# Starfish-develop/Starfish

Hardware: AMD Instinct MI355X
Metric: log-likelihood evals/sec, 4096-pixel order, batch=128 walkers (higher is better)
Workload: dtype f64; 1 GPU; cfg2: synthetic single order N_pix=4096, 8 eigenspectra, M=27, N_f=8192, 1 global + 1 local kernel, all 13 parameters thawed, batch=128 walkers per GPU; global_batch=128, units_per_gpu=128, parallelism=(order x walker) units sharded x1, one process per GPU, no data-path collective

## Files before the change

starfish_amd/csrc/sf_abi.cpp:

```cpp
#include "sf_stages.h"

sf_emu_args emu_args(sf_ctx* c, const sf_model_desc* mdl, const double* d_params, const Work& w, double* d_mu, double* d_cov,
                     double* d_Lw, int* d_info) {
    sf_emu_args e;
    e.params = d_params;
    e.pstride = sf_param_stride(c, mdl);
    e.off_grid = 6;
    e.m = c->m;
    e.M = c->M;
    e.P = c->P;
    e.grid = c->grid.as<double>();
    e.variances = c->variances.as<double>();
    e.lengthscales = c->lengthscales.as<double>();
    e.gmin = c->gmin.as<double>();
    e.gmax = c->gmax.as<double>();
    e.alpha = c->alpha.as<double>();
    e.LinvT = c->Linv.as<double>();
    e.zscratch = w.zs;
    e.kbuf = w.kv;
    e.mu = d_mu;
    e.cov = d_cov;
    e.Lw = d_Lw;
    e.info = d_info;
    return e;
// ... 256 lines not shown
    hipStream_t s = (hipStream_t)stream;
    prof_count_call();
    {
        ProfScope ps(s, PS_TRANSFORM);
        rc = run_transforms(c, mdl, B, d_params, w, nullptr, nullptr, nullptr, nullptr, true, s);
        if (rc) return rc;
    }
    {
        ProfScope ps(s, PS_FILL);
        rc = fill_dense(c, mdl, B, d_params, w, d_cov, ld, stride, lower_only ? 1 : 0, add_jitter ? 1 : 0, c->n, s);
        if (rc) return rc;
    }
    return export_info(d_info, w, B, s);
}

sf_fill_args loglike_fill_args(sf_ctx* c, const sf_model_desc* mdl, const double* d_params, const Work& w, const Layout& L,
                               int fp) {
    sf_fill_args f = fill_args(c, mdl, d_params, w);
    f.C = w.C;
    f.lda = L.lda;
    f.stride = (int64_t)L.npad * L.lda;
    f.lower_only = 1;
    f.add_jitter = 1;
    f.gtab = w.gtab;
    f.tilemap = w.tilemap;
    f.tilelist = w.tilelist;
    f.tilecount = w.tilecount;
    f.list_cap = (int)tilemap_bytes(L);
    f.fp = fp;
    f.nt128 = (L.npad + fp + 127) / 128;
    return f;
}
int loglike_factor_finish(const Work& w, const Layout& L, int fp, int units, double* ltbuf, double* d_lnl, int* d_info,
                          hipStream_t s, sf_exec* ex) {
    const int64_t stride = (int64_t)L.npad * L.lda;
    int rc;
    {
        ProfScope ps(s, PS_POTRF);
        sf_gen_args gen;
        gen.Y = w.Y;
        gen.mpad = L.mpad;
        gen.ldy = L.npad;
        gen.tilemap = w.tilemap;
        gen.fp = fp;
        gen.nt128 = (L.npad + fp + 127) / 128;
        rc = sf_launch_potrf(w.C, L.npad, L.lda, stride, units, w.info_c, ltbuf, w.resid, L.npad, s, &gen, ex);
        if (rc) return rc;
    }
    {
        ProfScope ps(s, PS_SOLVE);
        rc = sf_launch_logdet_z(w.C, L.npad, L.lda, stride, units, w.resid, L.npad, w.logdet, w.sqmah, s);
        if (rc) return rc;
        rc = sf_launch_finish(units, w.logdet, w.sqmah, w.info_e, w.info_c, d_lnl, d_info, s);
        if (rc) return rc;
    }
    return SF_OK;
}

extern "C" int sf_loglike_batch(sf_ctx* c, const sf_model_desc* mdl, int B, const double* d_params,
                                double* d_lnl, double* d_logdet, double* d_sqmah, double* d_resid,
                                double* d_log_scale, int* d_info, void* d_work, size_t work_bytes,
                                void* stream) {
    Work w;
    int rc = open_call(c, mdl, B, d_work, work_bytes, true, &w);
    if (rc) return rc;
    if (!d_lnl) {
        sf_set_error("sf_loglike_batch: d_lnl is required");
        return SF_EINVAL;
    }
    hipStream_t s = (hipStream_t)stream;
    prof_count_call();
    const Layout L = layout_of(c);
    {
        ProfScope ps(s, PS_TRANSFORM);
        rc = run_transforms(c, mdl, B, d_params, w, nullptr, nullptr, d_resid, d_log_scale, true, s);
        if (rc) return rc;
    }
    const int fp = sf_potrf_front_pad(c->npad, B);
    {
        ProfScope ps(s, PS_FILL);
        rc = sf_launch_fill(loglike_fill_args(c, mdl, d_params, w, L, fp), B, s);
        if (rc) return rc;
    }
    rc = loglike_factor_finish(w, L, fp, B, w.ltbuf, d_lnl, d_info, s, &c->exec);
    if (rc) return rc;
    return export_logdet_sqmah(d_logdet, d_sqmah, w, B, s);
}
```

starfish_amd/csrc/sf_chol_seq.h:

```cpp
#pragma once
#include "sf_chol_host.h"
#include "sf_chol_diag.h"
#include "sf_chol_panel.h"
#include "sf_chol_wide.h"

static int sf_check_front_pad(int fp, int n) {
    if (fp != 0 && (fp != 64 || n % GT != 64)) {
        sf_set_error("potrf: front pad %d does not fit n = %d", fp, n);
        return SF_EINVAL;
    }
    return SF_OK;
}

template <class Args>
static void sf_park(Args& g, const sf_potrf_scratch& ws) {
    g.Sout = ws.T;
    g.sS = ws.sT;
    g.ldS = SF_LDT;
}
static double sf_slab_rows(int n, int row0, int nslab, int step) {
    double rows = 0.0;
    for (int i = 0; i < nslab; ++i) {
        const int r0 = row0 + i * step * GT;
        rows += (n - r0 < GT) ? n - r0 : GT;
// ... 103 lines not shown
    g.slab_step = step;
    g.Wt0 = ws.Wslot(k);
    g.Wt1 = ws.Wslot(k + 1);
    g.sW = ws.sW;
    if (park) sf_park(g, ws);
    const long long nblk = (long long)nslab * batch;
    SF_TRY(sf_check_grid(nblk));
#ifdef SF_TUNING
    if (stamps.t && stamps.n < 64) {
        stamps.k[stamps.n] = k * 1000 + nslab;
        g.stamps = stamps.t + 16 * stamps.n++;
    }
#endif
    const double rows = sf_slab_rows(n, g.row0, nslab, step);
    const double kk = g.k0 > fp ? g.k0 - fp : 0;
    const double flops = (2.0 * kk * rows * GT + 2.0 * (kk + GT) * rows * GT + 2.0 * (rows * GT * (double)GT + (double)GT * rows * GT)) * batch;
    void* tok;
    sf_prof_gemm_begin(st, flops, &tok);
    if (g.rhs)
        hipLaunchKernelGGL(k_chol_panel_w<true>, dim3((unsigned)nblk), dim3(1024), SF_PANELW_LDS, st, g);
    else
        hipLaunchKernelGGL(k_chol_panel_w<false>, dim3((unsigned)nblk), dim3(1024), SF_PANELW_LDS, st, g);
    sf_prof_gemm_end(tok);
    SF_LAUNCH_CHECK();
    return SF_OK;
}

static int sf_diag_step(const sf_potrf_scratch& ws, double* A, int lda, int64_t stride, double* rhs, int ldr, int* info, int n, int k,
                        double* Wt, int fp, hipStream_t st) {
    const int k0 = k * GT;
    const int pw = (n - k0 < GT) ? n - k0 : GT;
    return sf_launch_diag128(ws.T, ws.sT, pw, info, k0 - fp, rhs ? rhs + k0 : nullptr, ldr, A + (int64_t)k0 * lda + k0, lda, stride, Wt,
                             ws.sW, ws.batch, st, k == 0 ? fp : 0);
}

struct sf_narrow_events {
    hipEvent_t d, rest[2];
};
static int sf_narrow_step(const sf_panel_args& base, const sf_potrf_scratch& ws, sf_exec* ex, int* info, int k, double* Wt, hipStream_t c,
                          const hipStream_t gs[2], const hipEvent_t last[2], hipEvent_t* e_top, sf_narrow_events* ev) {
    const int n = base.n, fp = base.fp, nt = (n + GT - 1) / GT;
    const int k0 = k * GT;
    const int pw = (n - k0 < GT) ? n - k0 : GT;
    *ev = {};
    SF_TRY(sf_diag_step(ws, base.C, base.lda, base.sC, base.rhs, base.ldr, info, n, k, Wt, fp, c));
    if (k + 1 >= nt) return SF_OK;
    SF_TRY(sf_exec_event(ex, &ev->d));
    SF_HIP(hipEventRecord(ev->d, c));
    const int gk = (k + 1) & 1;
    if (e_top && sf_panel_split(k0, pw, fp, ws.batch) > 1) {
        if (*e_top) SF_HIP(hipStreamWaitEvent(gs[gk], *e_top, 0));
        SF_TRY(sf_panel_step(base, ws, k0, pw, (k + 1) * GT, 1, 1, Wt, true, gs[gk], 0, 1));
        hipEvent_t e_part;
        SF_TRY(sf_exec_event(ex, &e_part));
        SF_HIP(hipEventRecord(e_part, gs[gk]));
        SF_HIP(hipStreamWaitEvent(c, e_part, 0));
        SF_TRY(sf_panel_step(base, ws, k0, pw, (k + 1) * GT, 1, 1, Wt, true, c, 0, 2));
    } else {
        if (last[gk]) SF_HIP(hipStreamWaitEvent(c, last[gk], 0));
        SF_TRY(sf_panel_step(base, ws, k0, pw, (k + 1) * GT, 1, 1, Wt, true, c, 0, 0));
    }
    if (e_top) {
        SF_TRY(sf_exec_event(ex, e_top));
        SF_HIP(hipEventRecord(*e_top, c));
    }
    for (int g = 0; g < 2; ++g) {
        const int first = k + 2 + (((k + 2) & 1) != g);
        if (first >= nt) continue;
        const int cnt = (nt - 1 - first) / 2 + 1;
        SF_HIP(hipStreamWaitEvent(gs[g], ev->d, 0));
        SF_TRY(sf_panel_step(base, ws, k0, pw, first * GT, cnt, 2, Wt, false, gs[g], 1 + g, 0));
        SF_TRY(sf_exec_event(ex, &ev->rest[g]));
        SF_HIP(hipEventRecord(ev->rest[g], gs[g]));
    }
    return SF_OK;
}

static int sf_launch_potrf_v2(double* A, int n, int lda, int64_t stride, int* info, const sf_potrf_scratch& ws, double* rhs,
                              int ldr, hipStream_t s, const sf_gen_args* gen, sf_exec* ex, int fp) {
    const int batch = ws.batch;
    SF_HIP(hipMemsetAsync(info, 0, sizeof(int) * (size_t)batch, s));
    SF_TRY(sf_exec_prepare(ex));
    constexpr int G = 2;
    hipStream_t c = ex->side;
    const hipStream_t gs[G] = {s, ex->grp[0]};
    SF_TRY(sf_exec_fork(ex, s, {c, gs[1]}));

    const sf_panel_args base = sf_panel_frame<sf_panel_args>(A, n, lda, stride, rhs, ldr, gen, fp);
    const int nt = (n + GT - 1) / GT;
    SF_TRY(sf_panel_step(base, ws, 0, 0, 0, 1, 1, nullptr, true, c, 0, 0));
    hipEvent_t e_epi = nullptr;
    hipEvent_t e_rest[G] = {};
    hipEvent_t e_rest_prev[G] = {};
    for (int k = 0; k < nt; ++k) {
        for (int g = 0; g < G; ++g)
            if (e_rest_prev[g]) SF_HIP(hipStreamWaitEvent(c, e_rest_prev[g], 0));
        sf_narrow_events ev;
        SF_TRY(sf_narrow_step(base, ws, ex, info, k, ws.Wbuf(k & 1), c, gs, e_rest, &e_epi, &ev));
        for (int g = 0; g < G; ++g) {
            e_rest_prev[g] = e_rest[g];
            if (ev.rest[g]) e_rest[g] = ev.rest[g];
        }
    }
    SF_TRY(sf_exec_join(ex, s, c, {e_rest[1]}));
    return SF_OK;
}

static int sf_launch_potrf_v3(double* A, int n, int lda, int64_t stride, int* info, const sf_potrf_scratch& ws, double* rhs,
                              int ldr, hipStream_t s, const sf_gen_args* gen, sf_exec* ex, bool half, int fp) {
    const int batch = ws.batch;
    static sf_dev_once attr_once;
    SF_CHECK(sf_lds_limit_once(&attr_once, 160 * 1024, {(const void*)k_chol_panel_w<true>, (const void*)k_chol_panel_w<false>}));
    SF_HIP(hipMemsetAsync(info, 0, sizeof(int) * (size_t)batch, s));
    SF_TRY(sf_exec_prepare(ex));
    hipStream_t c = ex->side, xa = ex->side;
    SF_TRY(sf_exec_fork(ex, s, {c, xa, ex->grp[0]}));
    const int nt = (n + GT - 1) / GT;

    const sf_panel_args base = sf_panel_frame<sf_panel_args>(A, n, lda, stride, rhs, ldr, gen, fp);
    const sf_panelw_args wbase = sf_panel_frame<sf_panelw_args>(A, n, lda, stride, rhs, ldr, gen, fp);
    sf_wide_stamps stamps;
    SF_TRY(sf_wide_stamps_begin(stamps));
    auto diag = [&](int k) -> int { return sf_diag_step(ws, A, lda, stride, rhs, ldr, info, n, k, ws.Wslot(k), fp, c); };

    SF_TRY(sf_panel_step(base, ws, 0, 0, 0, 1, 1, nullptr, true, c, 0, 0));
    const hipStream_t bs[2] = {s, ex->grp[0]};
    hipEvent_t e_A = nullptr;
    hipEvent_t e_last[2] = {nullptr, nullptr};
    std::vector<hipEvent_t> readers[4];
    auto wait_readers = [&](int slot) -> int {
        for (hipEvent_t e : readers[slot]) SF_HIP(hipStreamWaitEvent(c, e, 0));
        readers[slot].clear();
        return SF_OK;
    };
    int k = 0;
    for (; k < nt; k += 2) {
        if (k + 2 >= nt) break;
        if (half && k >= (nt / 4) * 2 && k > 0) break;
        if (e_A) SF_HIP(hipStreamWaitEvent(c, e_A, 0));
        SF_TRY(wait_readers(k & 3));
        SF_TRY(diag(k));
        SF_TRY(sf_panel_step(base, ws, k * GT, GT, (k + 1) * GT, 1, 1, ws.Wslot(k), true, c, 0, 0));
        SF_TRY(wait_readers((k + 1) & 3));
        SF_TRY(diag(k + 1));
        hipEvent_t e_chain;
        SF_TRY(sf_exec_event(ex, &e_chain));
        SF_HIP(hipEventRecord(e_chain, c));
        const int na = (nt - (k + 2) < 2) ? nt - (k + 2) : 2;
        SF_HIP(hipStreamWaitEvent(xa, e_chain, 0));
        for (int g = 0; g < 2; ++g)
            if (e_last[g]) SF_HIP(hipStreamWaitEvent(xa, e_last[g], 0));
        SF_TRY(sf_panel_step_w(wbase, ws, k, k + 2, na, 1, true, xa, stamps));
        SF_TRY(sf_exec_event(ex, &e_A));
        SF_HIP(hipEventRecord(e_A, xa));
        readers[k & 3].push_back(e_A);
        readers[(k + 1) & 3].push_back(e_A);
        for (int g = 0; g < 2; ++g) {
            const int first = k + 4 + g;
            if (first >= nt) continue;
            const int cnt = (nt - 1 - first) / 2 + 1;
            SF_HIP(hipStreamWaitEvent(bs[g], e_chain, 0));
            SF_TRY(sf_panel_step_w(wbase, ws, k, first, cnt, 2, false, bs[g], stamps));
            SF_TRY(sf_exec_event(ex, &e_last[g]));
            SF_HIP(hipEventRecord(e_last[g], bs[g]));
            readers[k & 3].push_back(e_last[g]);
            readers[(k + 1) & 3].push_back(e_last[g]);
        }
    }
    for (; k < nt; ++k) {
        if (e_A) {
            SF_HIP(hipStreamWaitEvent(c, e_A, 0));
            for (int g = 0; g < 2; ++g) SF_HIP(hipStreamWaitEvent(bs[g], e_A, 0));
            e_A = nullptr;
        }
        SF_TRY(wait_readers(k & 3));
        sf_narrow_events ev;
        SF_TRY(sf_narrow_step(base, ws, ex, info, k, ws.Wslot(k), c, bs, e_last, nullptr, &ev));
        for (int g = 0; g < 2; ++g)
            if (ev.rest[g]) {
                e_last[g] = ev.rest[g];
                readers[k & 3].push_back(ev.rest[g]);
            }
    }
    SF_TRY(sf_exec_join(ex, s, c, {e_A, e_last[1]}));
    sf_wide_stamps_report(stamps, s);
    return SF_OK;
}
```

starfish_amd/csrc/sf_common.h:

```cpp
#pragma once
#include <hip/hip_runtime.h>
#include <stdint.h>
#include <stddef.h>
#include <stdlib.h>
#include <atomic>
#include <initializer_list>
#include <mutex>
#include "sf_base.h"

#define SF_LEAF 64
#define SF_NB 256
#define SF_MAX_LOCAL 32
#define SF_NF_MIN_VSINI 16
#define SF_NF_MAX_VSINI 65536

typedef double sf_d4 __attribute__((ext_vector_type(4)));

#define SF_HIP(call)                                                                     \
    do {                                                                                 \
        hipError_t e_ = (call);                                                          \
        if (e_ != hipSuccess) {                                                          \
            sf_set_error("%s:%d %s -> %s", __FILE__, __LINE__, #call, hipGetErrorString(e_)); \
            return SF_EHIP;                                                              \
        }                                                                                \
// ... 28 lines not shown
}
static inline int sf_lds_limit_once(sf_dev_once* once, int bytes, std::initializer_list<const void*> kernels) {
    return sf_once_per_device(once, [&]() -> int {
        for (const void* k : kernels) SF_HIP(hipFuncSetAttribute(k, hipFuncAttributeMaxDynamicSharedMemorySize, bytes));
        return SF_OK;
    });
}
#define SF_CHECK(expr)              \
    do {                            \
        const int rc_ = (expr);     \
        if (rc_ != SF_OK) return rc_; \
    } while (0)

#ifdef SF_TUNING
#define SF_TUNE_FLAG(name) (getenv(name) != nullptr)
#define SF_TUNE_INT(name, dflt) (getenv(name) ? atoi(getenv(name)) : (dflt))
#define SF_TUNE_STR(name) (static_cast<const char*>(getenv(name)))
#else
#define SF_TUNE_FLAG(name) (false)
#define SF_TUNE_INT(name, dflt) (dflt)
#define SF_TUNE_STR(name) (static_cast<const char*>(nullptr))
#endif

#ifndef SF_EXEC_GROUPS
#define SF_EXEC_GROUPS 2
#endif
static_assert(SF_EXEC_GROUPS >= 2, "the wide sequence and the multi-order lanes use grp[0]: at least two slab groups");
struct sf_exec {
    int device = -1;
    hipStream_t side = nullptr;
    hipStream_t grp[SF_EXEC_GROUPS - 1] = {};
    hipStream_t aux = nullptr;
    hipEvent_t fork = nullptr, join = nullptr;
    hipEvent_t* pool = nullptr;
    size_t pool_size = 0, pool_cap = 0, used = 0;
};
int sf_exec_prepare(sf_exec* ex);
int sf_exec_event(sf_exec* ex, hipEvent_t* e);
void sf_exec_release(sf_exec* ex);
sf_exec* sf_exec_thread_local(void);

void sf_prof_gemm_begin(hipStream_t s, double flops, void** tok);
void sf_prof_gemm_end(void* tok);

#define SF_LTB_DOUBLES (SF_LEAF * SF_LEAF + SF_LEAF)
#define SF_LDT (SF_NB + 16)
size_t sf_potrf_work_doubles(int n, int batch);
struct sf_gen_args {
    const double* Y;
    int mpad, ldy;
    const unsigned char* tilemap;
    int nt128;
    int fp;
};
int sf_potrf_front_pad(int n, int batch);
int sf_launch_potrf(double* A, int n, int lda, int64_t stride, int batch, int* info, double* work,
                    double* rhs, int ldr, hipStream_t s, const sf_gen_args* gen = nullptr, sf_exec* ex = nullptr);
int sf_band_tiles_lda(int nband);
size_t sf_band_tiles_doubles(int nband, int batch);
int sf_band_tiles_wt(int halfwidth);
int sf_set_persistent_potrf(int enable);
int sf_persistent_potrf_read_status(long long* out8);
int sf_set_cholesky_sequence(int mode);
int sf_launch_logdet_z(const double* L, int n, int lda, int64_t stride, int batch, const double* z, int ldr,
                       double* logdet, double* sqmah, hipStream_t s);
int sf_launch_logdet_sqmah(const double* L, int n, int lda, int64_t stride, int batch,
                           const double* R, int ldr, double* zscratch, double* logdet, double* sqmah, hipStream_t s);
int sf_launch_chol_apply(const double* L, int n, int lda, int64_t stride, int batch, int op, const double* rhs, int nrhs,
                         int ldr, int64_t rhs_stride, double* out, int ldo, int64_t out_stride, hipStream_t s);
int sf_launch_apply_stage(const double* rhs, int ldr, int64_t rhs_stride, const double* resid, int n, int npad, int nrhs,
                          int batch, double* stage, hipStream_t s);
int sf_launch_apply_export(const double* stage, const int* info, int n, int npad, int nrhs, int batch, double* out,
                           hipStream_t s);
size_t sf_chol_inverse_work_doubles(int n, int batch);
int sf_launch_chol_inverse_diag(double* L, int n, int lda, int64_t stride, int batch, double* winv, double* out,
                                int64_t out_stride, hipStream_t s);
int sf_launch_diag_copy(const double* A, int n, int lda, int64_t stride, int batch, double* diag, hipStream_t s);

int sf_launch_clock_probe(long long* out, long long wall_ticks, hipStream_t s);

struct sf_fill_args {
    const double* wave;
    const double* sigma;
    const double* Y;
    const double* params;
    double* C;
    int n, npad, lda, mpad, ldy, pstride;
    int64_t stride;
    int has_global, n_local, off_global, off_local;
    int lower_only;
    int add_jitter;
    int nout;
    int monotonic;
    int loguniform;
    unsigned char* tilemap;
    int nt128;
    int fp;
    unsigned* tilelist;
    int* tilecount;
    int list_cap;
    double* gtab;
};
static inline __host__ __device__ int sf_fill_extent(const sf_fill_args& a) {
    return a.nout > 0 ? a.nout : (a.lower_only ? a.npad : a.n);
}
int sf_launch_fill(const sf_fill_args& a, int B, hipStream_t s);
size_t sf_fill_dense_map_tiles(int n);
int sf_launch_fill_dense(const sf_fill_args& a, int B, unsigned char* smap, unsigned short* list, int* count, hipStream_t s,
                         sf_exec* ex);
int sf_launch_stream_write(double* dst, size_t count, double v, hipStream_t s);
int sf_launch_cov_matvec(const sf_fill_args& f, int m, const double* v, int ldv, int nrhs, int batch, double* yv,
                         const int* info, double* out, hipStream_t s);
int sf_launch_cinv_blocks(const double* L, int n, int lda, int64_t stride, int batch, const double* winv, const int* pairs,
                          int npairs, double* out, hipStream_t s);
static inline __host__ __device__ int sf_cov_grad_slots(int has_global, int n_local) { return (has_global ? 2 : 0) + 3 * n_local; }
size_t sf_cov_grad_work_doubles(int n, int has_global, int n_local, int batch);
int sf_launch_cov_grad(const sf_fill_args& f, int batch, const double* winv, const double* alpha, int ld_alpha, const int* info,
                       double* part, double* grad, int grad_stride, hipStream_t s);
struct sf_multi_reduce_args {
    const double* unit_lnl;
    const int* unit_info;
    const double* unit_grad;
    const int* col_ptr;
    const int* col_src;
    int nseg, W, grad_stride, ncols, out_stride;
    double* lnl;
    double* grad;
    int* info;
};
int sf_launch_multi_grad_reduce(const sf_multi_reduce_args& a, hipStream_t s);
static inline __host__ __device__ int sf_emu_grad_slots(int m, int P) { return 1 + m + m * P; }
size_t sf_emu_grad_work_doubles(int M, int P, int m, int batch);
int sf_launch_emu_grad(const double* grid, int M, int P, int m, const double* hyper, int hyper_stride, int batch,
                       const double* iphiphi, const double* L, int npad, int lda, int64_t stride, const double* winv,
                       const double* alpha, int ld_alpha, const int* info, double* part, double* grad, int grad_stride,
                       hipStream_t s);
int sf_launch_band_fill(const sf_fill_args& a, int B, double* band, int ws, int halfwidth, int ldb, int64_t sband,
                        int* info, double* gtab, hipStream_t s, int tile_wt = -1);
int sf_launch_global_cov(const double* wave, int n, double amp, double ls, double* out, hipStream_t s);
// ... 43 lines not shown
```

starfish_amd/csrc/sf_exec.cpp:

```cpp
#include <cstdlib>

#include "sf_common.h"

int sf_exec_prepare(sf_exec* ex) {
    int dev = 0;
    SF_HIP(hipGetDevice(&dev));
    if (ex->side == nullptr || ex->device != dev) {
        if (ex->side) sf_exec_release(ex);
        int prio_lo = 0, prio_hi = 0;
        SF_HIP(hipDeviceGetStreamPriorityRange(&prio_lo, &prio_hi));
        SF_HIP(hipStreamCreateWithPriority(&ex->side, hipStreamNonBlocking, prio_hi));
        SF_HIP(hipStreamCreateWithPriority(&ex->aux, hipStreamNonBlocking, prio_hi));
        for (int g = 0; g < SF_EXEC_GROUPS - 1; ++g) SF_HIP(hipStreamCreateWithFlags(&ex->grp[g], hipStreamNonBlocking));
        SF_HIP(hipEventCreateWithFlags(&ex->fork, hipEventDisableTiming));
        SF_HIP(hipEventCreateWithFlags(&ex->join, hipEventDisableTiming));
        ex->device = dev;
    }
    ex->used = 0;
    return SF_OK;
}
int sf_exec_event(sf_exec* ex, hipEvent_t* e) {
    if (ex->used == ex->pool_size) {
        if (ex->pool_size == ex->pool_cap) {
            const size_t cap = ex->pool_cap ? 2 * ex->pool_cap : 256;
            hipEvent_t* np = (hipEvent_t*)realloc(ex->pool, cap * sizeof(hipEvent_t));
            if (!np) {
                sf_set_error("out of host memory (event pool)");
                return SF_ENOMEM;
            }
            ex->pool = np;
            ex->pool_cap = cap;
        }
        hipEvent_t ne;
        SF_HIP(hipEventCreateWithFlags(&ne, hipEventDisableTiming));
        ex->pool[ex->pool_size++] = ne;
    }
    *e = ex->pool[ex->used++];
    return SF_OK;
}
void sf_exec_release(sf_exec* ex) {
    if (!ex) return;
    for (size_t i = 0; i < ex->pool_size; ++i) (void)hipEventDestroy(ex->pool[i]);
    free(ex->pool);
    ex->pool = nullptr;
    ex->pool_size = ex->pool_cap = ex->used = 0;
    if (ex->fork) (void)hipEventDestroy(ex->fork);
    if (ex->join) (void)hipEventDestroy(ex->join);
    if (ex->side) (void)hipStreamDestroy(ex->side);
    if (ex->aux) (void)hipStreamDestroy(ex->aux);
    for (int g = 0; g < SF_EXEC_GROUPS - 1; ++g) {
        if (ex->grp[g]) (void)hipStreamDestroy(ex->grp[g]);
        ex->grp[g] = nullptr;
    }
    ex->fork = ex->join = nullptr;
    ex->side = ex->aux = nullptr;
    ex->device = -1;
}
sf_exec* sf_exec_thread_local(void) {
    static thread_local sf_exec per_device[64];
    int dev = 0;
    (void)hipGetDevice(&dev);
    return &per_device[(dev >= 0 && dev < 64) ? dev : 0];
}
```

starfish_amd/csrc/sf_fill_elem.h:

```cpp
#pragma once

__device__ __forceinline__ double sf_matern_elem(double w_row, double w_col, double amp, double ls,
                                                 double r0) {
    const double r = SF_C_KMS / 2 * fabs((w_col - w_row) / (w_col + w_row));
    if (!(r <= r0)) return 0.0;
    const double taper = 0.5 + 0.5 * cos(M_PI * r / r0);
    const double s3 = 1.7320508075688772;
    return taper * amp * (1 + s3 * r / ls) * exp(-s3 * r / ls);
}

__device__ __forceinline__ double sf_local_elem(double d_row, double d_col, double amp, double sigma,
                                                double r0) {
    const double r_tap = fmax(d_col, d_row);
    if (!(r_tap <= r0)) return 0.0;
    const double r2 = d_col * d_col + d_row * d_row;
    const double taper = 0.5 + 0.5 * cos(M_PI * r_tap / r0);
    return taper * amp * exp(-0.5 * r2 / (sigma * sigma));
}

__device__ __forceinline__ double sf_local_metric(double w, double mu) {
    return SF_C_KMS / mu * fabs(w - mu);
}

struct sf_global_hyper {
    double amp, ls, r0;
};
__device__ __forceinline__ sf_global_hyper sf_load_global(const sf_fill_args& a, const double* __restrict__ P) {
    sf_global_hyper g;
    g.amp = exp(P[a.off_global]);
    g.ls = exp(P[a.off_global + 1]);
    g.r0 = 6 * g.ls;
    return g;
}
struct sf_local_hyper {
    double mu, amp, sig;
};
__device__ __forceinline__ sf_local_hyper sf_load_local(const sf_fill_args& a, const double* __restrict__ P, int k) {
    sf_local_hyper l;
    l.mu = P[a.off_local + 3 * k];
    l.amp = exp(P[a.off_local + 3 * k + 1]);
    l.sig = exp(P[a.off_local + 3 * k + 2]);
    return l;
}

__device__ __forceinline__ void sf_block_support(const sf_fill_args& a, const double* __restrict__ P, int rlo, int rhi,
                                                 int clo, int chi, double g_r0, bool& do_glob, unsigned& lmask) {
    const bool on_diag = !(rlo > chi || clo > rhi);
    do_glob = false;
    lmask = 0;
    if (a.has_global) {
        do_glob = true;
        if (a.monotonic && !on_diag) {
            double wr, wc;
            if (rlo > chi) { wr = a.wave[rlo]; wc = a.wave[chi]; }
            else { wr = a.wave[rhi]; wc = a.wave[clo]; }
            const double rmin = SF_C_KMS / 2 * fabs((wc - wr) / (wc + wr));
            do_glob = rmin <= g_r0 * (1 + 1e-9);
        }
    }
    for (int k = 0; k < a.n_local; ++k) {
        bool hit = true;
        if (a.monotonic) {
            const sf_local_hyper l = sf_load_local(a, P, k);
            const double mu = l.mu, r0 = 4 * l.sig;
            auto dmin = [&](int lo, int hi) {
                const double wl = a.wave[lo], wh = a.wave[hi];
                if (wl <= mu && mu <= wh) return 0.0;
                return fmin(sf_local_metric(wl, mu), sf_local_metric(wh, mu));
            };
            hit = (dmin(rlo, rhi) <= r0 * (1 + 1e-9)) && (dmin(clo, chi) <= r0 * (1 + 1e-9));
        }
        if (hit) lmask |= 1u << k;
    }
}

static int sf_check_n_local(const sf_fill_args& a) {
    if (a.n_local > SF_MAX_LOCAL) {
        sf_set_error("at most %d local kernels are supported", SF_MAX_LOCAL);
        return SF_EINVAL;
    }
    return SF_OK;
}
static int sf_check_fill_grid(long long nblk) {
    if (nblk > 0x7fffffffLL) {
        sf_set_error("fill grid too large");
        return SF_EINVAL;
    }
    return SF_OK;
}
```

starfish_amd/csrc/sf_fill_tile.h:

```cpp
#pragma once

#define FT 64

__device__ __forceinline__ void sf_rank_m_subtile(const sf_fill_args& a, const double* __restrict__ Yb, int R0, int C0,
                                                  sf_d4 (&acc)[2][2]) {
    const int lane = threadIdx.x & 63;
    const int gam = lane & 15, q = lane >> 4;
#pragma unroll
    for (int i = 0; i < 2; ++i)
#pragma unroll
        for (int j = 0; j < 2; ++j) acc[i][j] = (sf_d4){0.0, 0.0, 0.0, 0.0};
    const int colperm = 4 * (gam & 3) + (gam >> 2);
    for (int kk = 0; kk < a.mpad; kk += 4) {
        const double* yk = Yb + (int64_t)(kk + q) * a.ldy;
        double brow[2], acol[2];
#pragma unroll
        for (int i = 0; i < 2; ++i) {
            brow[i] = yk[R0 + i * 16 + gam];
            acol[i] = yk[C0 + i * 16 + colperm];
        }
#pragma unroll
        for (int i = 0; i < 2; ++i)
#pragma unroll
            for (int j = 0; j < 2; ++j)
// ... 65 lines not shown
                        const double d_row = sf_local_metric(w_row, l.mu);
#pragma unroll
                        for (int r = 0; r < 4; ++r)
                            loc[r] = loc[r] + sf_local_elem(d_row, sf_local_metric(w_col[r], l.mu), l.amp, l.sig, 4 * l.sig);
                    }
#pragma unroll
                    for (int r = 0; r < 4; ++r)
                        if (col0 + r < a.n) v[r] = v[r] + loc[r];
                }
            }
            if (a.add_jitter && row < a.n) {
#pragma unroll
                for (int r = 0; r < 4; ++r)
                    if (col0 + r == row) v[r] = v[r] + SF_JITTER;
            }
            double* dst = Cb + (int64_t)row * a.lda + col0;
            if (vec_ok && col0 + 3 < nout) {
                *(double2*)dst = make_double2(v[0], v[1]);
                *(double2*)(dst + 2) = make_double2(v[2], v[3]);
            } else {
#pragma unroll
                for (int r = 0; r < 4; ++r)
                    if (col0 + r < nout) dst[r] = v[r];
            }
            if (mirror) {
#pragma unroll
                for (int r = 0; r < 4; ++r)
                    if (col0 + r < nout) Cb[(int64_t)(col0 + r) * a.lda + row] = v[r];
            }
        }
    }
}

template <bool BAND>
__device__ __forceinline__ void sf_fill_tile(const sf_fill_args& a, int b, int tm, int tn) {
    if (a.lower_only && tn > tm) return;
    if (a.tilemap) {
        const int fs = a.fp >> 6;
        if (!a.tilemap[(int64_t)b * a.nt128 * a.nt128 + ((tm + fs) >> 1) * a.nt128 + ((tn + fs) >> 1)]) return;
    }

    const int w = threadIdx.x >> 6;
    const int R0 = tm * FT + (w >> 1) * 32, C0 = tn * FT + (w & 1) * 32;
    const int nout = sf_fill_extent(a);
    if (R0 >= nout || C0 >= nout) return;
    if (a.lower_only && C0 > R0 + 31) return;
    const double* __restrict__ Yb = a.Y + (int64_t)b * a.mpad * a.ldy;
    sf_d4 acc[2][2];
    sf_rank_m_subtile(a, Yb, R0, C0, acc);
    sf_tile_finish<BAND>(a, b, R0, C0, acc);
}

__global__ __launch_bounds__(256) void k_tile_map(sf_fill_args a) {
    const int nt = a.nt128;
    const int e = blockIdx.x * 256 + threadIdx.x, b = blockIdx.y;
    if (e >= nt * nt) return;
    const int tm = e / nt, tn = e - tm * nt;
    unsigned char flag = 0;
    if (tn <= tm) {
        const int vr = tm * 128, vc = tn * 128;
        const int rlo = max(vr - a.fp, 0), clo = max(vc - a.fp, 0);
        if (vr / SF_NB == vc / SF_NB || rlo >= a.n) {
            flag = 1;
        } else {
            const int rhi = min(vr - a.fp + 127, a.n - 1), chi = min(vc - a.fp + 127, a.n - 1);
            const double* __restrict__ P = a.params + (int64_t)b * a.pstride;
            bool do_glob;
            unsigned lmask;
            sf_block_support(a, P, rlo, rhi, clo, chi, a.has_global ? sf_load_global(a, P).r0 : 0.0, do_glob, lmask);
            flag = (do_glob || lmask) ? 1 : 0;
        }
    }
    a.tilemap[(int64_t)b * nt * nt + e] = flag;
    if (flag && a.tilelist) {
        const int idx = atomicAdd(&a.tilecount[b], 1);
        if (idx < a.list_cap) a.tilelist[(int64_t)b * a.list_cap + idx] = ((unsigned)tm << 16) | (unsigned)tn;
    }
}

template <bool BAND>
__global__ __launch_bounds__(256, BAND ? 2 : 4) void k_fill_tiles(sf_fill_args a, int nt) {
    const int id = sf_xcd_remap(blockIdx.x, gridDim.x);
    const int tiles = nt * nt;
    const int b = id / tiles;
    const int t = id - b * tiles;
    sf_fill_tile<BAND>(a, b, t / nt, t - (t / nt) * nt);
}
template <bool BAND>
__global__ __launch_bounds__(256, BAND ? 2 : 4) void k_fill_tiles_list(sf_fill_args a, int G) {
    const int b = blockIdx.x / G, g = blockIdx.x - b * G;
    const int cnt = min(a.tilecount[b], a.list_cap) * 4;
    const unsigned* __restrict__ list = a.tilelist + (int64_t)b * a.list_cap;
    const int fs = a.fp >> 6;
    for (int li = g; li < cnt; li += G) {
        const unsigned e = list[li >> 2];
        const int tm = 2 * (int)(e >> 16) + ((li >> 1) & 1) - fs, tn = 2 * (int)(e & 0xffff) + (li & 1) - fs;
        if (tm >= 0 && tn >= 0) sf_fill_tile<BAND>(a, b, tm, tn);
    }
}

int sf_launch_fill(const sf_fill_args& a, int B, hipStream_t s) {
    SF_CHECK(sf_check_n_local(a));
    if (a.fp != 0 && (a.fp != 64 || !a.tilemap || !a.lower_only)) {
        sf_set_error("fill: a shifted tile frame needs fp = 64, a tile map and lower_only");
        return SF_EINVAL;
    }
    const int nout = sf_fill_extent(a);
    const int nt = (nout + FT - 1) / FT;
    const long long nblk = (long long)nt * nt * B;
    SF_CHECK(sf_check_fill_grid(nblk));
    const bool listed = a.tilemap && a.tilelist && a.tilecount && a.lower_only;
    if (a.tilemap) {
        if (listed) SF_HIP(hipMemsetAsync(a.tilecount, 0, sizeof(int) * (size_t)B, s));
        hipLaunchKernelGGL(k_tile_map, dim3((a.nt128 * a.nt128 + 255) / 256, B), dim3(256), 0, s, a);
        SF_LAUNCH_CHECK();
    }
    const int structured = a.has_global || a.n_local > 0;
    sf_fill_args a2 = a;
    if (!(a.gtab && a.has_global && a.loguniform && a.lower_only)) a2.gtab = nullptr;
    if (a2.gtab) {
        hipLaunchKernelGGL(k_band_gtab, dim3((a.n + 255) / 256, B), dim3(256), 0, s, a, a2.gtab, a.n - 1);
        SF_LAUNCH_CHECK();
    }
    if (listed) {
        const int G = 64;
        if (structured) hipLaunchKernelGGL(k_fill_tiles_list<true>, dim3((unsigned)B * G), dim3(256), 0, s, a2, G);
        else hipLaunchKernelGGL(k_fill_tiles_list<false>, dim3((unsigned)B * G), dim3(256), 0, s, a2, G);
    } else if (structured) hipLaunchKernelGGL(k_fill_tiles<true>, dim3((unsigned)nblk), dim3(256), 0, s, a2, nt);
    else hipLaunchKernelGGL(k_fill_tiles<false>, dim3((unsigned)nblk), dim3(256), 0, s, a2, nt);
    SF_LAUNCH_CHECK();
    return SF_OK;
}
```

starfish_amd/csrc/sf_stages.h:

```cpp
#pragma once
#include "sf_prof.h"
#include "sf_work.h"

#pragma GCC visibility push(hidden)
int open_call(const sf_ctx* c, const sf_model_desc* mdl, int B, void* d_work, size_t have, bool need_C, Work* w);
int run_transforms(sf_ctx* c, const sf_model_desc* mdl, int B, const double* d_params, const Work& w, double* d_flux_out,
                   double* d_X_out, double* d_resid_out, double* d_log_scale, bool want_Y, hipStream_t s);
sf_emu_args emu_args(sf_ctx* c, const sf_model_desc* mdl, const double* d_params, const Work& w, double* d_mu, double* d_cov,
                     double* d_Lw, int* d_info);
sf_broaden_args broaden_args(sf_ctx* c, const sf_model_desc* mdl, int B, const double* d_params, const Work& w);
sf_eval_args eval_args(sf_ctx* c, const sf_model_desc* mdl, const double* d_params, const Work& w);
sf_fill_args fill_args(sf_ctx* c, const sf_model_desc* mdl, const double* d_params, const Work& w);
sf_fill_args loglike_fill_args(sf_ctx* c, const sf_model_desc* mdl, const double* d_params, const Work& w, const Layout& L, int fp);
int loglike_factor_finish(const Work& w, const Layout& L, int fp, int units, double* ltbuf, double* d_lnl, int* d_info,
                          hipStream_t s, sf_exec* ex);
int export_info(int* d_info, const Work& w, int units, hipStream_t s);
int export_logdet_sqmah(double* d_logdet, double* d_sqmah, const Work& w, int units, hipStream_t s);
int mean_slots_ok(const char* who, const sf_ctx* c, const sf_model_desc* mdl, const int* h_slots, int nslots, int grad_stride);
sf_mean_grad_args mean_grad_kernel_args(const sf_ctx* c, const int* h_slots, int nslots, const Work& w, const AppliedWork& aw,
                                        double* d_grad, int grad_stride);
#pragma GCC visibility pop
```

Before: 2771 evals/s.

## Split covariance fill into map/head/bulk phases overlapped with transforms and Cholesky

Measured after the change: 2780 evals/s, median of 6. No clear change (+0.3%).

```diff
diff --git a/starfish_amd/csrc/sf_abi.cpp b/starfish_amd/csrc/sf_abi.cpp
--- a/starfish_amd/csrc/sf_abi.cpp
+++ b/starfish_amd/csrc/sf_abi.cpp
@@ -312,7 +312,7 @@
     return f;
 }
 int loglike_factor_finish(const Work& w, const Layout& L, int fp, int units, double* ltbuf, double* d_lnl, int* d_info,
-                          hipStream_t s, sf_exec* ex) {
+                          hipStream_t s, sf_exec* ex, hipEvent_t head_ready) {
     const int64_t stride = (int64_t)L.npad * L.lda;
     int rc;
     {
@@ -324,6 +324,7 @@
         gen.tilemap = w.tilemap;
         gen.fp = fp;
         gen.nt128 = (L.npad + fp + 127) / 128;
+        gen.head_ready = head_ready;
         rc = sf_launch_potrf(w.C, L.npad, L.lda, stride, units, w.info_c, ltbuf, w.resid, L.npad, s, &gen, ex);
         if (rc) return rc;
     }
@@ -351,18 +352,31 @@
     hipStream_t s = (hipStream_t)stream;
     prof_count_call();
     const Layout L = layout_of(c);
+    sf_exec* ex = &c->exec;
+    rc = sf_exec_prepare(ex);
+    if (rc) return rc;
+    const int fp = sf_potrf_front_pad(c->npad, B);
+    const sf_fill_args fa = loglike_fill_args(c, mdl, d_params, w, L, fp);
+    SF_HIP(hipEventRecord(ex->fork, s));
+    SF_HIP(hipStreamWaitEvent(ex->aux, ex->fork, 0));
+    rc = sf_launch_fill(fa, B, ex->aux, SF_FILL_MAP);
+    if (rc) return rc;
+    SF_HIP(hipEventRecord(ex->join, ex->aux));
     {
         ProfScope ps(s, PS_TRANSFORM);
         rc = run_transforms(c, mdl, B, d_params, w, nullptr, nullptr, d_resid, d_log_scale, true, s);
         if (rc) return rc;
     }
-    const int fp = sf_potrf_front_pad(c->npad, B);
     {
         ProfScope ps(s, PS_FILL);
-        rc = sf_launch_fill(loglike_fill_args(c, mdl, d_params, w, L, fp), B, s);
-        if (rc) return rc;
-    }
-    rc = loglike_factor_finish(w, L, fp, B, w.ltbuf, d_lnl, d_info, s, &c->exec);
+        SF_HIP(hipStreamWaitEvent(s, ex->join, 0));
+        rc = sf_launch_fill(fa, B, s, SF_FILL_HEAD);
+        if (rc) return rc;
+        SF_HIP(hipEventRecord(ex->head, s));
+        rc = sf_launch_fill(fa, B, s, SF_FILL_BULK);
+        if (rc) return rc;
+    }
+    rc = loglike_factor_finish(w, L, fp, B, w.ltbuf, d_lnl, d_info, s, ex, ex->head);
     if (rc) return rc;
     return export_logdet_sqmah(d_logdet, d_sqmah, w, B, s);
 }
diff --git a/starfish_amd/csrc/sf_chol_seq.h b/starfish_amd/csrc/sf_chol_seq.h
--- a/starfish_amd/csrc/sf_chol_seq.h
+++ b/starfish_amd/csrc/sf_chol_seq.h
@@ -159,6 +159,25 @@
     const int pw = (n - k0 < GT) ? n - k0 : GT;
     return sf_launch_diag128(ws.T, ws.sT, pw, info, k0 - fp, rhs ? rhs + k0 : nullptr, ldr, A + (int64_t)k0 * lda + k0, lda, stride, Wt,
                              ws.sW, ws.batch, st, k == 0 ? fp : 0);
+}
+
+static int sf_seq_start(sf_exec* ex, hipStream_t s, hipStream_t c, std::initializer_list<hipStream_t> others, int* info, int batch,
+                        const sf_gen_args* gen, hipEvent_t* e_bulk) {
+    hipEvent_t e;
+    SF_TRY(sf_exec_event(ex, &e));
+    const hipEvent_t head = gen ? gen->head_ready : nullptr;
+    if (head) SF_HIP(hipStreamWaitEvent(c, head, 0));
+    SF_HIP(hipMemsetAsync(info, 0, sizeof(int) * (size_t)batch, head ? c : s));
+    SF_HIP(hipEventRecord(e, s));
+    if (!head) SF_HIP(hipStreamWaitEvent(c, e, 0));
+    for (hipStream_t t : others) SF_HIP(hipStreamWaitEvent(t, e, 0));
+    *e_bulk = head ? e : nullptr;
+    return SF_OK;
+}
+static int sf_seq_bulk_wait(hipStream_t c, hipEvent_t* e_bulk) {
+    if (*e_bulk) SF_HIP(hipStreamWaitEvent(c, *e_bulk, 0));
+    *e_bulk = nullptr;
+    return SF_OK;
 }
 
 struct sf_narrow_events {
@@ -206,12 +225,12 @@
 static int sf_launch_potrf_v2(double* A, int n, int lda, int64_t stride, int* info, const sf_potrf_scratch& ws, double* rhs,
                               int ldr, hipStream_t s, const sf_gen_args* gen, sf_exec* ex, int fp) {
     const int batch = ws.batch;
-    SF_HIP(hipMemsetAsync(info, 0, sizeof(int) * (size_t)batch, s));
     SF_TRY(sf_exec_prepare(ex));
     constexpr int G = 2;
     hipStream_t c = ex->side;
     const hipStream_t gs[G] = {s, ex->grp[0]};
-    SF_TRY(sf_exec_fork(ex, s, {c, gs[1]}));
+    hipEvent_t e_bulk;
+    SF_TRY(sf_seq_start(ex, s, c, {gs[1]}, info, batch, gen, &e_bulk));
 
     const sf_panel_args base = sf_panel_frame<sf_panel_args>(A, n, lda, stride, rhs, ldr, gen, fp);
     const int nt = (n + GT - 1) / GT;
@@ -224,6 +243,7 @@
             if (e_rest_prev[g]) SF_HIP(hipStreamWaitEvent(c, e_rest_prev[g], 0));
         sf_narrow_events ev;
         SF_TRY(sf_narrow_step(base, ws, ex, info, k, ws.Wbuf(k & 1), c, gs, e_rest, &e_epi, &ev));
+        SF_TRY(sf_seq_bulk_wait(c, &e_bulk));
         for (int g = 0; g < G; ++g) {
             e_rest_prev[g] = e_rest[g];
             if (ev.rest[g]) e_rest[g] = ev.rest[g];
@@ -238,10 +258,10 @@
     const int batch = ws.batch;
     static sf_dev_once attr_once;
     SF_CHECK(sf_lds_limit_once(&attr_once, 160 * 1024, {(const void*)k_chol_panel_w<true>, (const void*)k_chol_panel_w<false>}));
-    SF_HIP(hipMemsetAsync(info, 0, sizeof(int) * (size_t)batch, s));
     SF_TRY(sf_exec_prepare(ex));
     hipStream_t c = ex->side, xa = ex->side;
-    SF_TRY(sf_exec_fork(ex, s, {c, xa, ex->grp[0]}));
+    hipEvent_t e_bulk;
+    SF_TRY(sf_seq_start(ex, s, c, {ex->grp[0]}, info, batch, gen, &e_bulk));
     const int nt = (n + GT - 1) / GT;
 
     const sf_panel_args base = sf_panel_frame<sf_panel_args>(A, n, lda, stride, rhs, ldr, gen, fp);
@@ -273,6 +293,7 @@
         hipEvent_t e_chain;
         SF_TRY(sf_exec_event(ex, &e_chain));
         SF_HIP(hipEventRecord(e_chain, c));
+        SF_TRY(sf_seq_bulk_wait(c, &e_bulk));
         const int na = (nt - (k + 2) < 2) ? nt - (k + 2) : 2;
         SF_HIP(hipStreamWaitEvent(xa, e_chain, 0));
         for (int g = 0; g < 2; ++g)
@@ -303,6 +324,7 @@
         SF_TRY(wait_readers(k & 3));
         sf_narrow_events ev;
         SF_TRY(sf_narrow_step(base, ws, ex, info, k, ws.Wslot(k), c, bs, e_last, nullptr, &ev));
+        SF_TRY(sf_seq_bulk_wait(c, &e_bulk));
         for (int g = 0; g < 2; ++g)
             if (ev.rest[g]) {
                 e_last[g] = ev.rest[g];
diff --git a/starfish_amd/csrc/sf_common.h b/starfish_amd/csrc/sf_common.h
--- a/starfish_amd/csrc/sf_common.h
+++ b/starfish_amd/csrc/sf_common.h
@@ -84,6 +84,7 @@
     hipStream_t grp[SF_EXEC_GROUPS - 1] = {};
     hipStream_t aux = nullptr;
     hipEvent_t fork = nullptr, join = nullptr;
+    hipEvent_t head = nullptr;
     hipEvent_t* pool = nullptr;
     size_t pool_size = 0, pool_cap = 0, used = 0;
 };
@@ -104,6 +105,7 @@
     const unsigned char* tilemap;
     int nt128;
     int fp;
+    hipEvent_t head_ready = nullptr;
 };
 int sf_potrf_front_pad(int n, int batch);
 int sf_launch_potrf(double* A, int n, int lda, int64_t stride, int batch, int* info, double* work,
@@ -156,7 +158,8 @@
 static inline __host__ __device__ int sf_fill_extent(const sf_fill_args& a) {
     return a.nout > 0 ? a.nout : (a.lower_only ? a.npad : a.n);
 }
-int sf_launch_fill(const sf_fill_args& a, int B, hipStream_t s);
+enum { SF_FILL_MAP = 1, SF_FILL_HEAD = 2, SF_FILL_BULK = 4, SF_FILL_ALL = 7 };
+int sf_launch_fill(const sf_fill_args& a, int B, hipStream_t s, int parts = SF_FILL_ALL);
 size_t sf_fill_dense_map_tiles(int n);
 int sf_launch_fill_dense(const sf_fill_args& a, int B, unsigned char* smap, unsigned short* list, int* count, hipStream_t s,
                          sf_exec* ex);
diff --git a/starfish_amd/csrc/sf_exec.cpp b/starfish_amd/csrc/sf_exec.cpp
--- a/starfish_amd/csrc/sf_exec.cpp
+++ b/starfish_amd/csrc/sf_exec.cpp
@@ -14,6 +14,7 @@
         for (int g = 0; g < SF_EXEC_GROUPS - 1; ++g) SF_HIP(hipStreamCreateWithFlags(&ex->grp[g], hipStreamNonBlocking));
         SF_HIP(hipEventCreateWithFlags(&ex->fork, hipEventDisableTiming));
         SF_HIP(hipEventCreateWithFlags(&ex->join, hipEventDisableTiming));
+        SF_HIP(hipEventCreateWithFlags(&ex->head, hipEventDisableTiming));
         ex->device = dev;
     }
     ex->used = 0;
@@ -46,13 +47,14 @@
     ex->pool_size = ex->pool_cap = ex->used = 0;
     if (ex->fork) (void)hipEventDestroy(ex->fork);
     if (ex->join) (void)hipEventDestroy(ex->join);
+    if (ex->head) (void)hipEventDestroy(ex->head);
     if (ex->side) (void)hipStreamDestroy(ex->side);
     if (ex->aux) (void)hipStreamDestroy(ex->aux);
     for (int g = 0; g < SF_EXEC_GROUPS - 1; ++g) {
         if (ex->grp[g]) (void)hipStreamDestroy(ex->grp[g]);
         ex->grp[g] = nullptr;
     }
-    ex->fork = ex->join = nullptr;
+    ex->fork = ex->join = ex->head = nullptr;
     ex->side = ex->aux = nullptr;
     ex->device = -1;
 }
diff --git a/starfish_amd/csrc/sf_fill_elem.h b/starfish_amd/csrc/sf_fill_elem.h
--- a/starfish_amd/csrc/sf_fill_elem.h
+++ b/starfish_amd/csrc/sf_fill_elem.h
@@ -43,8 +43,9 @@
     return l;
 }
 
-__device__ __forceinline__ void sf_block_support(const sf_fill_args& a, const double* __restrict__ P, int rlo, int rhi,
-                                                 int clo, int chi, double g_r0, bool& do_glob, unsigned& lmask) {
+template <class W, class L>
+__device__ __forceinline__ void sf_block_support_from(const sf_fill_args& a, W&& wave_at, L&& local_at, int rlo, int rhi, int clo,
+                                                      int chi, double g_r0, bool& do_glob, unsigned& lmask) {
     const bool on_diag = !(rlo > chi || clo > rhi);
     do_glob = false;
     lmask = 0;
@@ -52,8 +53,8 @@
         do_glob = true;
         if (a.monotonic && !on_diag) {
             double wr, wc;
-            if (rlo > chi) { wr = a.wave[rlo]; wc = a.wave[chi]; }
-            else { wr = a.wave[rhi]; wc = a.wave[clo]; }
+            if (rlo > chi) { wr = wave_at(rlo); wc = wave_at(chi); }
+            else { wr = wave_at(rhi); wc = wave_at(clo); }
             const double rmin = SF_C_KMS / 2 * fabs((wc - wr) / (wc + wr));
             do_glob = rmin <= g_r0 * (1 + 1e-9);
         }
@@ -61,10 +62,10 @@
     for (int k = 0; k < a.n_local; ++k) {
         bool hit = true;
         if (a.monotonic) {
-            const sf_local_hyper l = sf_load_local(a, P, k);
+            const sf_local_hyper l = local_at(k);
             const double mu = l.mu, r0 = 4 * l.sig;
             auto dmin = [&](int lo, int hi) {
-                const double wl = a.wave[lo], wh = a.wave[hi];
+                const double wl = wave_at(lo), wh = wave_at(hi);
                 if (wl <= mu && mu <= wh) return 0.0;
                 return fmin(sf_local_metric(wl, mu), sf_local_metric(wh, mu));
             };
@@ -72,6 +73,11 @@
         }
         if (hit) lmask |= 1u << k;
     }
+}
+__device__ __forceinline__ void sf_block_support(const sf_fill_args& a, const double* __restrict__ P, int rlo, int rhi,
+                                                 int clo, int chi, double g_r0, bool& do_glob, unsigned& lmask) {
+    sf_block_support_from(a, [&](int i) { return a.wave[i]; }, [&](int k) { return sf_load_local(a, P, k); }, rlo, rhi, clo, chi,
+                          g_r0, do_glob, lmask);
 }
 
 static int sf_check_n_local(const sf_fill_args& a) {
diff --git a/starfish_amd/csrc/sf_fill_tile.h b/starfish_amd/csrc/sf_fill_tile.h
--- a/starfish_amd/csrc/sf_fill_tile.h
+++ b/starfish_amd/csrc/sf_fill_tile.h
@@ -121,6 +121,43 @@
     }
 }
 
+__device__ __forceinline__ void sf_tile_sum4_table(const sf_fill_args& a, int row, int col0, const sf_d4& acc, double sg, bool table,
+                                                   const double (&gt)[4], double (&v)[4]) {
+#pragma unroll
+    for (int r = 0; r < 4; ++r) {
+        const int col = col0 + r;
+        double val = acc[r];
+        if (row < a.n && col < a.n) {
+            if (row == col) val = val + sg * sg;
+        } else {
+            val = (row == col) ? 1.0 : 0.0;
+        }
+        v[r] = val;
+    }
+    if (table && row < a.n) {
+#pragma unroll
+        for (int r = 0; r < 4; ++r)
+            if (col0 + r < a.n) v[r] = v[r] + gt[r];
+    }
+    if (a.add_jitter && row < a.n) {
+#pragma unroll
+        for (int r = 0; r < 4; ++r)
+            if (col0 + r == row) v[r] = v[r] + SF_JITTER;
+    }
+}
+__device__ __forceinline__ void sf_tile_store4(const sf_fill_args& a, double* Cb, int row, int col0, const double (&v)[4], int nout,
+                                               bool vec_ok) {
+    double* dst = Cb + (int64_t)row * a.lda + col0;
+    if (vec_ok && col0 + 3 < nout) {
+        *(double2*)dst = make_double2(v[0], v[1]);
+        *(double2*)(dst + 2) = make_double2(v[2], v[3]);
+    } else {
+#pragma unroll
+        for (int r = 0; r < 4; ++r)
+            if (col0 + r < nout) dst[r] = v[r];
+    }
+}
+
 template <bool BAND>
 __device__ __forceinline__ void sf_fill_tile(const sf_fill_args& a, int b, int tm, int tn) {
     if (a.lower_only && tn > tm) return;
@@ -139,6 +176,9 @@
     sf_rank_m_subtile(a, Yb, R0, C0, acc);
     sf_tile_finish<BAND>(a, b, R0, C0, acc);
 }
+
+#define SF_TILE_NONE 0xffffffffu
+__host__ __device__ static inline int sf_tile_head_slots(int nt128) { return nt128 >= 2 ? 3 : 1; }
 
 __global__ __launch_bounds__(256) void k_tile_map(sf_fill_args a) {
     const int nt = a.nt128;
@@ -161,9 +201,15 @@
         }
     }
     a.tilemap[(int64_t)b * nt * nt + e] = flag;
-    if (flag && a.tilelist) {
-        const int idx = atomicAdd(&a.tilecount[b], 1);
-        if (idx < a.list_cap) a.tilelist[(int64_t)b * a.list_cap + idx] = ((unsigned)tm << 16) | (unsigned)tn;
+    if (a.tilelist && tn <= tm) {
+        unsigned* __restrict__ list = a.tilelist + (int64_t)b * a.list_cap;
+        const unsigned entry = ((unsigned)tm << 16) | (unsigned)tn;
+        if (tm < 2) {
+            list[tm + tn] = flag ? entry : SF_TILE_NONE;
+        } else if (flag) {
+            const int idx = sf_tile_head_slots(nt) + atomicAdd(&a.tilecount[b], 1);
+            if (idx < a.list_cap) list[idx] = entry;
+        }
     }
 }
 
@@ -175,20 +221,181 @@
     const int t = id - b * tiles;
     sf_fill_tile<BAND>(a, b, t / nt, t - (t / nt) * nt);
 }
+struct sf_tile_ahead {
+    unsigned e_next;
+    bool ok;
+    int Rt, Ct, R0, C0;
+    double brow[2][2], acol[2][2];
+    double wr, wc, sgl, gtl;
+};
 template <bool BAND>
-__global__ __launch_bounds__(256, BAND ? 2 : 4) void k_fill_tiles_list(sf_fill_args a, int G) {
+__global__ __launch_bounds__(256, 3) void k_fill_tiles_list(sf_fill_args a, int G, int first, int nfixed, int counted) {
+    __shared__ double s_r0;
+    __shared__ double s_loc[BAND ? SF_MAX_LOCAL : 1][3];
     const int b = blockIdx.x / G, g = blockIdx.x - b * G;
-    const int cnt = min(a.tilecount[b], a.list_cap) * 4;
-    const unsigned* __restrict__ list = a.tilelist + (int64_t)b * a.list_cap;
+    const int tid = threadIdx.x, lane = tid & 63, w = tid >> 6;
+    const int gam = lane & 15, q = lane >> 4;
+    if (BAND) {
+        const double* __restrict__ P = a.params + (int64_t)b * a.pstride;
+        if (tid < a.n_local) {
+            const sf_local_hyper l = sf_load_local(a, P, tid);
+            s_loc[tid][0] = l.mu, s_loc[tid][1] = l.amp, s_loc[tid][2] = l.sig;
+        }
+        if (tid == 64 && a.has_global) s_r0 = sf_load_global(a, P).r0;
+        __syncthreads();
+    }
+    auto local_at = [&](int k) { return sf_local_hyper{s_loc[k][0], s_loc[k][1], s_loc[k][2]}; };
+    const int cnt = 4 * (nfixed + (counted ? max(0, min(a.tilecount[b], a.list_cap - first - nfixed)) : 0));
+    if (g >= cnt) return;
+    const unsigned* list = a.tilelist + (int64_t)b * a.list_cap + first;
     const int fs = a.fp >> 6;
-    for (int li = g; li < cnt; li += G) {
-        const unsigned e = list[li >> 2];
+    const int nout = sf_fill_extent(a);
+    const bool vec_ok = ((a.lda | a.stride) & 1) == 0;
+    const int nk = a.mpad >> 2;
+    const bool y_ahead = a.mpad <= 8;
+    const double* Yb = a.Y + (int64_t)b * a.mpad * a.ldy;
+    const double* gtb = (BAND && a.gtab) ? a.gtab + (int64_t)b * a.n : nullptr;
+    double* Cb = a.C + (int64_t)b * a.stride;
+    const int colperm = 4 * (gam & 3) + (gam >> 2);
+
+    sf_tile_ahead t;
+    sf_d4 acc[2][2];
+    auto request = [&](int li) {
+        const unsigned e = t.e_next;
+        t.e_next = (li + G < cnt) ? list[(li + G) >> 2] : SF_TILE_NONE;
         const int tm = 2 * (int)(e >> 16) + ((li >> 1) & 1) - fs, tn = 2 * (int)(e & 0xffff) + (li & 1) - fs;
-        if (tm >= 0 && tn >= 0) sf_fill_tile<BAND>(a, b, tm, tn);
-    }
-}
-
-int sf_launch_fill(const sf_fill_args& a, int B, hipStream_t s) {
+        t.Rt = tm * FT, t.Ct = tn * FT;
+        t.R0 = t.Rt + (w >> 1) * 32, t.C0 = t.Ct + (w & 1) * 32;
+        t.ok = e != SF_TILE_NONE && tm >= 0 && tn >= 0 && !(a.lower_only && tn > tm) && t.R0 < nout && t.C0 < nout &&
+               !(a.lower_only && t.C0 > t.R0 + 31);
+        if (!t.ok) return;
+        if (y_ahead) {
+#pragma unroll
+            for (int k = 0; k < 2; ++k)
+                if (k < nk) {
+                    const double* yk = Yb + (int64_t)(4 * k + q) * a.ldy;
+#pragma unroll
+                    for (int i = 0; i < 2; ++i) {
+                        t.brow[k][i] = yk[t.R0 + i * 16 + gam];
+                        t.acol[k][i] = yk[t.C0 + i * 16 + colperm];
+                    }
+                }
+        }
+        t.wr = t.wc = 1.0;
+        if (BAND) {
+            if (t.Rt + lane < a.n) t.wr = a.wave[t.Rt + lane];
+            if (t.Ct + lane < a.n) t.wc = a.wave[t.Ct + lane];
+        }
+        t.sgl = (tm == tn && t.Rt + lane < a.n) ? a.sigma[t.Rt + lane] : 0.0;
+        t.gtl = 0.0;
+        if (gtb) {
+            const int d = abs(t.R0 - t.C0 - 31 + lane);
+            if (lane < 63 && d < a.n) t.gtl = gtb[d];
+        }
+    };
+    auto rank_m = [&]() {
+        if (!y_ahead) return sf_rank_m_subtile(a, Yb, t.R0, t.C0, acc);
+#pragma unroll
+        for (int i = 0; i < 2; ++i)
+#pragma unroll
+            for (int j = 0; j < 2; ++j) acc[i][j] = (sf_d4){0.0, 0.0, 0.0, 0.0};
+#pragma unroll
+        for (int k = 0; k < 2; ++k)
+            if (k < nk) {
+#pragma unroll
+                for (int i = 0; i < 2; ++i)
+#pragma unroll
+                    for (int j = 0; j < 2; ++j)
+                        acc[i][j] = __builtin_amdgcn_mfma_f64_16x16x4f64(t.acol[k][j], t.brow[k][i], acc[i][j], 0, 0, 0);
+            }
+    };
+
+    t.e_next = list[g >> 2];
+    request(g);
+    if (t.ok) rank_m();
+    unsigned long long later = 0;
+    int it = 0;
+    for (int li = g;;) {
+        const bool ok = t.ok;
+        const int R0 = t.R0, C0 = t.C0;
+        double v[2][2][4];
+        bool deferred = false;
+        if (ok) {
+            const int Rt = t.Rt, Ct = t.Ct;
+            bool do_glob = false;
+            unsigned lmask = 0;
+            if (BAND && R0 < a.n && C0 < a.n) {
+                auto wave_at = [&](int i) {
+                    const bool r = (unsigned)(i - Rt) < (unsigned)FT;
+                    return __shfl(r ? t.wr : t.wc, r ? i - Rt : i - Ct);
+                };
+                sf_block_support_from(a, wave_at, local_at, R0, min(R0 + 31, a.n - 1), C0, min(C0 + 31, a.n - 1), a.has_global ? s_r0 : 0.0, do_glob,
+                                      lmask);
+            }
+            const bool table = BAND && do_glob && gtb;
+            deferred = !(BAND && (lmask || (do_glob && !gtb)));
+            if (!deferred) {
+                if (it < 64) later |= 1ull << it;
+            } else {
+#pragma unroll
+                for (int ti = 0; ti < 2; ++ti) {
+                    const int row = R0 + ti * 16 + gam;
+                    const double sg = __shfl(t.sgl, R0 - Rt + ti * 16 + gam);
+#pragma unroll
+                    for (int tj = 0; tj < 2; ++tj) {
+                        const int col0 = C0 + tj * 16 + 4 * q;
+                        double gt[4];
+#pragma unroll
+                        for (int r = 0; r < 4; ++r) gt[r] = table ? __shfl(t.gtl, (ti - tj) * 16 + gam - 4 * q - r + 31) : 0.0;
+                        if (row < nout && col0 < nout) sf_tile_sum4_table(a, row, col0, acc[ti][tj], sg, table, gt, v[ti][tj]);
+                    }
+                }
+            }
+        }
+        li += G;
+        const bool more = li < cnt;
+        if (more) {
+            request(li);
+            if (t.ok) rank_m();
+        }
+        if (deferred) {
+#pragma unroll
+            for (int ti = 0; ti < 2; ++ti) {
+                const int row = R0 + ti * 16 + gam;
+#pragma unroll
+                for (int tj = 0; tj < 2; ++tj) {
+                    const int col0 = C0 + tj * 16 + 4 * q;
+                    if (row < nout && col0 < nout) sf_tile_store4(a, Cb, row, col0, v[ti][tj], nout, vec_ok);
+                }
+            }
+        }
+        if (!more) break;
+        ++it;
+    }
+    if constexpr (BAND) {
+        const double* __restrict__ P = a.params + (int64_t)b * a.pstride;
+        it = 0;
+        for (int li = g; li < cnt; li += G, ++it) {
+            if (it < 64 && !((later >> it) & 1)) continue;
+            const unsigned e = list[li >> 2];
+            const int tm = 2 * (int)(e >> 16) + ((li >> 1) & 1) - fs, tn = 2 * (int)(e & 0xffff) + (li & 1) - fs;
+            const int R0 = tm * FT + (w >> 1) * 32, C0 = tn * FT + (w & 1) * 32;
+            if (it >= 64) {
+                if (e == SF_TILE_NONE || tm < 0 || tn < 0 || (a.lower_only && tn > tm) || R0 >= nout || C0 >= nout ||
+                    (a.lower_only && C0 > R0 + 31) || R0 >= a.n || C0 >= a.n)
+                    continue;
+                bool do_glob;
+                unsigned lmask;
+                sf_block_support(a, P, R0, min(R0 + 31, a.n - 1), C0, min(C0 + 31, a.n - 1), a.has_global ? s_r0 : 0.0, do_glob, lmask);
+                if (!(lmask || (do_glob && !gtb))) continue;
+            }
+            sf_rank_m_subtile(a, Yb, R0, C0, acc);
+            sf_tile_finish<true>(a, b, R0, C0, acc);
+        }
+    }
+}
+
+int sf_launch_fill(const sf_fill_args& a, int B, hipStream_t s, int parts) {
     SF_CHECK(sf_check_n_local(a));
     if (a.fp != 0 && (a.fp != 64 || !a.tilemap || !a.lower_only)) {
         sf_set_error("fill: a shifted tile frame needs fp = 64, a tile map and lower_only");
@@ -199,23 +406,41 @@
     const long long nblk = (long long)nt * nt * B;
     SF_CHECK(sf_check_fill_grid(nblk));
     const bool listed = a.tilemap && a.tilelist && a.tilecount && a.lower_only;
-    if (a.tilemap) {
-        if (listed) SF_HIP(hipMemsetAsync(a.tilecount, 0, sizeof(int) * (size_t)B, s));
-        hipLaunchKernelGGL(k_tile_map, dim3((a.nt128 * a.nt128 + 255) / 256, B), dim3(256), 0, s, a);
-        SF_LAUNCH_CHECK();
-    }
     const int structured = a.has_global || a.n_local > 0;
     sf_fill_args a2 = a;
     if (!(a.gtab && a.has_global && a.loguniform && a.lower_only)) a2.gtab = nullptr;
-    if (a2.gtab) {
-        hipLaunchKernelGGL(k_band_gtab, dim3((a.n + 255) / 256, B), dim3(256), 0, s, a, a2.gtab, a.n - 1);
+    if (!listed) {
+        a2.tilelist = nullptr;
+        if (!(parts & SF_FILL_BULK)) return SF_OK;
+        parts = SF_FILL_ALL;
+    }
+    if (parts & SF_FILL_MAP) {
+        if (a.tilemap) {
+            if (listed) SF_HIP(hipMemsetAsync(a.tilecount, 0, sizeof(int) * (size_t)B, s));
+            hipLaunchKernelGGL(k_tile_map, dim3((a.nt128 * a.nt128 + 255) / 256, B), dim3(256), 0, s, a2);
+            SF_LAUNCH_CHECK();
+        }
+        if (a2.gtab) {
+            hipLaunchKernelGGL(k_band_gtab, dim3((a.n + 255) / 256, B), dim3(256), 0, s, a, a2.gtab, a.n - 1);
+            SF_LAUNCH_CHECK();
+        }
+    }
+    if (listed) {
+        const int nh = sf_tile_head_slots(a.nt128);
+        auto list_fill = [&](int G, int first, int nfixed, int counted) {
+            if (structured)
+                hipLaunchKernelGGL(k_fill_tiles_list<true>, dim3((unsigned)B * G), dim3(256), 0, s, a2, G, first, nfixed, counted);
+            else
+                hipLaunchKernelGGL(k_fill_tiles_list<false>, dim3((unsigned)B * G), dim3(256), 0, s, a2, G, first, nfixed, counted);
+        };
+        const bool head = parts & SF_FILL_HEAD, bulk = (parts & SF_FILL_BULK) && a.list_cap > nh;
+        if (head && bulk) list_fill(64, 0, nh, 1);
+        else if (head) list_fill(4 * nh, 0, nh, 0);
+        else if (bulk) list_fill(64, nh, 0, 1);
         SF_LAUNCH_CHECK();
-    }
-    if (listed) {
-        const int G = 64;
-        if (structured) hipLaunchKernelGGL(k_fill_tiles_list<true>, dim3((unsigned)B * G), dim3(256), 0, s, a2, G);
-        else hipLaunchKernelGGL(k_fill_tiles_list<false>, dim3((unsigned)B * G), dim3(256), 0, s, a2, G);
-    } else if (structured) hipLaunchKernelGGL(k_fill_tiles<true>, dim3((unsigned)nblk), dim3(256), 0, s, a2, nt);
+        return SF_OK;
+    }
+    if (structured) hipLaunchKernelGGL(k_fill_tiles<true>, dim3((unsigned)nblk), dim3(256), 0, s, a2, nt);
     else hipLaunchKernelGGL(k_fill_tiles<false>, dim3((unsigned)nblk), dim3(256), 0, s, a2, nt);
     SF_LAUNCH_CHECK();
     return SF_OK;
diff --git a/starfish_amd/csrc/sf_stages.h b/starfish_amd/csrc/sf_stages.h
--- a/starfish_amd/csrc/sf_stages.h
+++ b/starfish_amd/csrc/sf_stages.h
@@ -13,7 +13,7 @@
 sf_fill_args fill_args(sf_ctx* c, const sf_model_desc* mdl, const double* d_params, const Work& w);
 sf_fill_args loglike_fill_args(sf_ctx* c, const sf_model_desc* mdl, const double* d_params, const Work& w, const Layout& L, int fp);
 int loglike_factor_finish(const Work& w, const Layout& L, int fp, int units, double* ltbuf, double* d_lnl, int* d_info,
-                          hipStream_t s, sf_exec* ex);
+                          hipStream_t s, sf_exec* ex, hipEvent_t head_ready = nullptr);
 int export_info(int* d_info, const Work& w, int units, hipStream_t s);
 int export_logdet_sqmah(double* d_logdet, double* d_sqmah, const Work& w, int units, hipStream_t s);
 int mean_slots_ok(const char* who, const sf_ctx* c, const sf_model_desc* mdl, const int* h_slots, int nslots, int grad_stride);
```
